# OEmiliatanO/Unpaired-Multimodal-Learning

Measured on AMD Instinct MI355X. Metric: samples/sec (img+text feats) UML head fine-tune, batch 4096, 1/2/4/8 GPU, higher is better.
Workload: dtype bf16; 1 GPU; cfg2 ImageNet-1k CLIP-ViT-B/16 features (d=512) + unpaired CUPL text, linear head C=1000, 4096 img + 4096 txt rows/step/GPU, scale 100, zero-shot init, AdamW lr 1e-3 wd 0.01, warm-up 50 + cosine 12800; n_img_rows=1281167, n_txt_rows=29940, global_batch=8192, parallelism=dp1, dp_stepping=single gpu, precision_mode=bf16, order_rng=device, steps_per_call=25

## Files before the change

### include/umlh.h

```cpp
#ifndef UMLH_H
#define UMLH_H

#include <stdint.h>

#ifdef __cplusplus
extern "C" {
#endif

#define UMLH_OK              0
#define UMLH_E_INVALID      -1
#define UMLH_E_UNBOUND      -2
#define UMLH_E_HIP          -3
#define UMLH_E_NOGPU        -4

#define UMLH_OPT_SGD   0
#define UMLH_OPT_ADAM  1
#define UMLH_OPT_ADAMW 2

#define UMLH_PREC_FP32 0
#define UMLH_PREC_BF16 1

typedef struct umlh_handle_s* umlh_handle_t;

typedef struct {
// ... 186 lines not shown
int  umlh_encoder_stack_backward(const umlh_enc_layer_t* cfg, int32_t n_layers, const float* const* P, const float* h0,
                                 const int64_t* lengths, const float* saved, const float* h, const float* dh_out, float* scratch,
                                 float* const* G, float* dh, float* dh0, void* stream);

typedef struct umlh_enc_plan_s* umlh_enc_plan_t;
uint64_t umlh_encoder_plan_floats(const umlh_enc_layer_t* cfg, int32_t n_layers);
int  umlh_encoder_plan_create(const umlh_enc_layer_t* cfg, int32_t n_layers, const float* const* P, int32_t has_lengths,
                              float* workspace, umlh_enc_plan_t* out);
int  umlh_encoder_plan_offsets(umlh_enc_plan_t plan, uint64_t offsets[6]);
int  umlh_encoder_plan_forward(umlh_enc_plan_t plan, uint64_t seed, void* stream);
int  umlh_encoder_plan_backward(umlh_enc_plan_t plan, void* stream);
void umlh_encoder_plan_destroy(umlh_enc_plan_t plan);

int  umlh_random_permutation(int64_t n, uint64_t seed, int64_t* out, void* stream);

int  umlh_optimizer_step(int32_t optimizer, float* param, const float* grad, float* m, float* v, int64_t n,
                         double lr, int64_t step, double beta1, double beta2, double eps, double momentum,
                         double weight_decay, void* stream);
int  umlh_optimizer_step_multi(int32_t optimizer, int32_t n_tensors, float* const* params, const float* const* grads,
                               float* const* m, float* const* v, const int64_t* n, double lr, int64_t step, double beta1,
                               double beta2, double eps, double momentum, double weight_decay, void* stream);


uint64_t umlh_align_scratch_bytes(int64_t n, int32_t d_a, int32_t d_b, int32_t topk, int32_t splits);
int  umlh_align_knn(const float* x, int64_t n, int32_t d, int32_t ldx, int32_t topk, int32_t splits, int32_t* knn,
                    float* scores, void* scratch, uint64_t scratch_bytes, void* stream);
int  umlh_align_mutual_knn(const int32_t* knn_a, const int32_t* knn_b, int64_t n, int32_t topk, double* out, void* scratch,
                           uint64_t scratch_bytes, void* stream);
int  umlh_align_cka(const float* a, int32_t lda, int32_t d_a, const float* b, int32_t ldb, int32_t d_b, int64_t n,
                    int32_t splits, double* out4, void* scratch, uint64_t scratch_bytes, void* stream);
// ... 138 lines not shown
```

### unpaired-multimodal-learning_amd/csrc/umlh_common.h

```cpp
#pragma once
#include <hip/hip_runtime.h>
#include <stdint.h>
#include "umlh.h"
#include <cstdlib>

typedef float f32x16 __attribute__((ext_vector_type(16)));
typedef float f32x4v __attribute__((ext_vector_type(4)));

constexpr int UMLH_MULTI_OPT_MAX = 48;

constexpr int KT = 16;

static inline int env_int(const char* name, int def) {
    const char* e = getenv(name);
    return e ? atoi(e) : def;
}
#if defined(__HIPCC__)
__device__ __forceinline__ void store_wt_f32(float* p, float v) {
    asm volatile("global_store_dword %0, %1, off sc1" ::"v"(p), "v"(v) : "memory");
}
__device__ __forceinline__ void store_out_f32x4(float* p, f32x4v v, int plain) {
    if (plain) *reinterpret_cast<f32x4v*>(p) = v;
    else asm volatile("global_store_dwordx4 %0, %1, off sc1" ::"v"(p), "v"(v) : "memory");
}
// ... 153 lines not shown
    int   M, N, K, lda, ldo, k_chunk, k_switch, k_valid1, k_valid2, nsplit;
    int   nsplit1;
    const int64_t* a_rows;
    int   bcs;
    void* out16;
    long long slab_stride;
    unsigned long long* stamps;
};

constexpr int UMLH_MULTI_REDUCE_MAX = 16;
struct ReduceDesc { const float* src; float* dst; long long stride; long long n; int ns; int blk0; };
struct MultiReduceArgs {
    ReduceDesc d[UMLH_MULTI_REDUCE_MAX]; int count;
    const float* s_num; const float* s_den; float s_mul;
};

struct OptArgs {
    int   kind;
    float lr, decay;
    float neg_step_size;
    float bc2_sqrt;
    float beta1, one_m_beta1, beta2, one_m_beta2, eps, momentum, wd;
    int   plain;
    int   x3;
};

struct FinalizeArgs {
    const float* partials;
    int   nb0, nb1;
    float inv_rows0, inv_rows1;
// ... 211 lines not shown
```

### unpaired-multimodal-learning_amd/csrc/umlh_kernels_f32.hip

```cpp
#include "umlh_common.h"
#include "umlh_launch.h"
#include <cstdlib>

#ifdef UMLH_ABLATIONS
#define UMLH_ABL(cond) (cond)
#else
#define UMLH_ABL(cond) (false)
#endif

__device__ __forceinline__ f32x4v load4_guard(const float* p, int lim, bool vec_ok) {
    f32x4v v = {0.f, 0.f, 0.f, 0.f};
    if (lim >= 4 && vec_ok) {
        v = *reinterpret_cast<const f32x4v*>(p);
    } else {
        if (lim > 0) v[0] = p[0];
        if (lim > 1) v[1] = p[1];
        if (lim > 2) v[2] = p[2];
        if (lim > 3) v[3] = p[3];
    }
    return v;
}

template <int CTW, int WC, int MODE>
__global__ __launch_bounds__(512) void fwd_ce_f32(FwdArgs a) {
// ... 1395 lines not shown
    for (int j = tid; j < d; j += 256) {
        float mean = count > 0 ? zsum[j] / (float)count : 0.f;
        zsum[j] = mean;
        ss += mean * mean;
    }
    redn[tid] = ss;
    __syncthreads();
    for (int off = 128; off > 0; off >>= 1) {
        if (tid < off) redn[tid] += redn[tid + off];
        __syncthreads();
    }
    float nrm = fmaxf(sqrtf(redn[0]), 1e-12f);
    for (int j = tid; j < d; j += 256) w[(size_t)c * d + j] = zsum[j] / nrm;
}

__device__ __forceinline__ unsigned mix32(unsigned x) {
    x ^= x >> 16; x *= 0x7feb352dU; x ^= x >> 15; x *= 0x846ca68bU; x ^= x >> 16;
    return x;
}

__global__ __launch_bounds__(256) void feistel_perm_kernel(long long n, unsigned long long seed, int half,
                                                           long long* __restrict__ out) {
    long long i = (long long)blockIdx.x * 256 + threadIdx.x;
    if (i >= n) return;
    const unsigned long long mask = (1ULL << half) - 1ULL;
    const unsigned k0 = (unsigned)seed, k1 = (unsigned)(seed >> 32);
    unsigned long long x = (unsigned long long)i;
    do {
        unsigned long long L = x >> half, R = x & mask;
#pragma unroll
        for (int r = 0; r < 4; ++r) {
            unsigned long long F = (unsigned long long)mix32((unsigned)R * 0x9e3779b1U + (r & 1 ? k1 : k0) + 0x85ebca6bU * (unsigned)r +
                                                               (unsigned)(R >> 32)) & mask;
            unsigned long long nl = R;
            R = L ^ F;
            L = nl;
        }
        x = (L << half) | R;
    } while (x >= (unsigned long long)n);
    out[i] = (long long)x;
}

__global__ __launch_bounds__(256) void w_shadow32_kernel(const float* __restrict__ w, float* __restrict__ dst, int C, int K, int cpad) {
    const long long q = (long long)blockIdx.x * 256 + threadIdx.x;
    const int tiles = cpad / 32;
    const long long total = (long long)(K / 16) * tiles * 128;
    if (q >= total) return;
    const int half = (int)(q & 1), lane = (int)((q >> 1) & 63);
    const int tile = (int)((q >> 7) % tiles), c = (int)((q >> 7) / tiles);
    const int cls = tile * 32 + (lane & 31);
    f32x4v v = {0.f, 0.f, 0.f, 0.f};
    if (cls < C) v = *reinterpret_cast<const f32x4v*>(w + (size_t)cls * K + c * 16 + 8 * (lane >> 5) + 4 * half);
    *reinterpret_cast<f32x4v*>(dst + q * 4) = v;
}

// ... 165 lines not shown
    long long n4 = (long long)hf->C * hf->K / 4;
    int blocks = (int)((n4 + 255) / 256) + 1;
    DiagArgs d = *dg;
    if (d.dst && (!d.part || !d.ticket)) return (int)hipErrorInvalidValue;
    if (d.n_slabs_img > hf->n_slabs) d.n_slabs_img = hf->n_slabs;
    OptArgs oc = hf->o;
    oc.plain = umlh_plain_stores();
    oc.x3 = umlh_f32_x3();
    hipLaunchKernelGGL(head_step_kernel, dim3(blocks), dim3(256), 0, stream, hf->slabs, hf->n_slabs, hf->slab_stride, hf->C, hf->K,
                       hf->p, hf->m, hf->v, oc, hf->shadow, hf->cpad, hf->f, hf->grad_out, d, shadow32);
    return (int)hipGetLastError();
}

int umlh_launch_feistel_perm(long long n, unsigned long long seed, long long* out, hipStream_t stream) {
    if (n <= 0) return 0;
    int bits = 1;
    while ((1LL << bits) < n) ++bits;
    int half = (bits + 1) / 2;
    hipLaunchKernelGGL(feistel_perm_kernel, dim3((unsigned)((n + 255) / 256)), dim3(256), 0, stream, n, seed, half, out);
    return (int)hipGetLastError();
}

int umlh_launch_finalize(const FinalizeArgs* f, hipStream_t stream) {
    hipLaunchKernelGGL(finalize_kernel, dim3(1), dim3(256), 0, stream, *f);
    return (int)hipGetLastError();
}

int umlh_launch_zero_shot(const float* feats, const int64_t* labels, long long n, int d, int C, float* w,
                          hipStream_t stream) {
    size_t sm = sizeof(float) * (size_t)(d + 256);
    hipLaunchKernelGGL(zero_shot_kernel, dim3(C), dim3(256), sm, stream, feats, labels, n, d, w);
    return (int)hipGetLastError();
}

// ... 2 lines not shown
```

### unpaired-multimodal-learning_amd/csrc/umlh_launch.h

```cpp
#pragma once
#include <atomic>
#include "umlh_common.h"
#include "umlh_micro.h"

inline long long align_up(long long x) { return (x + 255) / 256 * 256; }
template <class T>
inline T* at(void* scratch, long long off) { return reinterpret_cast<T*>(static_cast<char*>(scratch) + off); }

template <auto Kernel>
__attribute__((visibility("hidden"))) int raise_lds_limit(int bytes) {
    static std::atomic<unsigned long long> done{0};
    int dev = 0;
    hipError_t e = hipGetDevice(&dev);
    if (e != hipSuccess) return (int)e;
    if (!((done.load(std::memory_order_acquire) >> (dev & 63)) & 1ULL)) {
        e = hipFuncSetAttribute(reinterpret_cast<const void*>(Kernel), hipFuncAttributeMaxDynamicSharedMemorySize, bytes);
        if (e != hipSuccess) return (int)e;
        done.fetch_or(1ULL << (dev & 63), std::memory_order_release);
    }
    return 0;
}

extern "C" {
int umlh_launch_w_shadow32(const float* w, float* dst, int C, int K, int cpad, hipStream_t stream);
int umlh_f32_fwd_config(int C, int* ctw, int* wc);
int umlh_f32_launch_fwd(const FwdArgs* a, int ctw, int wc, int grid, hipStream_t stream);
int umlh_f32_launch_gemm(const GemmArgs* g, int ta, int tb, int splits, hipStream_t stream);
int umlh_f32_launch_gemm_enc(const GemmArgs* g, int ta, int tb, int splits, hipStream_t stream);
int umlh_launch_reduce_update(int mode, const float* slabs, int n_slabs, long long slab_stride, long long n, float* grad_out,
                              float* p, float* m, float* v, const OptArgs* o, long long frozen_lo, long long frozen_hi,
                              hipStream_t stream);
int umlh_launch_multi_opt(int n, float* const* p, const float* const* g, float* const* m, float* const* v, const long long* cnt,
                          const OptArgs* o, hipStream_t stream);
int umlh_launch_head_step(const HeadFuse* hf, const DiagArgs* dg, float* shadow32, hipStream_t stream);
int umlh_launch_feistel_perm(long long n, unsigned long long seed, long long* out, hipStream_t stream);
int umlh_launch_finalize(const FinalizeArgs* f, hipStream_t stream);
int umlh_launch_zero_shot(const float* feats, const int64_t* labels, long long n, int d, int C, float* w, hipStream_t stream);
int umlh_launch_to_bf16(const float* src, void* dst, long long n, hipStream_t stream);
int umlh_launch_iota(long long* dst, long long n, hipStream_t stream);
int umlh_launch_w_shadow(const float* w, void* dst, int C, int K, int cpad, hipStream_t stream);
int umlh_bf16_fwd_ts(int wc, int stw);
int umlh_bf16_launch_fwd_q(const FwdArgsB* a, int nq, int tiles, hipStream_t stream);
int umlh_bf16_launch_fwd(const FwdArgsB* a, int ctw, int wc, int stw, int grid, hipStream_t stream);
int umlh_bf16_launch_transpose_shadow(const float* src, int R, int Cc, int ldd, void* dst, int mode, hipStream_t stream);
int umlh_bf16_step_tasks(int nfwd, int M, int N, int splits, long long n_head, int with_head);
int umlh_bf16_launch_step(const FwdArgsB* a, int ctw, int wc, int nfwd, const DwArgsB* g, int splits, unsigned* claim,
                          unsigned long long* done, unsigned* status, unsigned epoch, int ts, int total_cols,
                          const HeadFuse* hf, unsigned long long* timeline, int cus, int lazy, hipStream_t stream);
int umlh_bf16_launch_dw(const DwArgsB* g, int splits, int am, int om, hipStream_t stream);
int umlh_micro_chunking(int d, int* nch, int* cw);
// ... 143 lines not shown
```

### unpaired-multimodal-learning_amd/csrc/umlh_ops.cpp

```cpp
#include <hip/hip_runtime.h>
#include <algorithm>
#include <cmath>
#include <cstring>

#include "umlh_host.h"
#include "umlh_launch.h"

static const int64_t ROWS_END = (int64_t)1 << 31;
static const int64_t ALIGN_MAX_ROWS = (int64_t)1 << 30;
static const int LIST_MAX_K = 24;

static_assert(sizeof(long long) == sizeof(int64_t), "the launchers' long long is the ABI's int64_t");
static inline const long long* ll(const int64_t* p) { return reinterpret_cast<const long long*>(p); }
static inline long long* ll(int64_t* p) { return reinterpret_cast<long long*>(p); }

static const char SCRATCH_OF[] = "%s: scratch of %llu bytes, %llu needed";
static const char SCRATCH_BYTES_EQ[] = "%s: scratch_bytes=%llu, %llu needed";
static int check_scratch(const char* who, const void* scratch, uint64_t scratch_bytes, uint64_t need, unsigned align,
                         const char* size_fmt = SCRATCH_OF) {
    if (scratch_bytes < need) return fail(UMLH_E_INVALID, size_fmt, who, (unsigned long long)scratch_bytes, (unsigned long long)need);
    if (align && (reinterpret_cast<uintptr_t>(scratch) & (align - 1)) != 0)
        return fail(UMLH_E_INVALID, "%s: scratch must be %u-byte aligned", who, align);
    return UMLH_OK;
}
// ... 233 lines not shown
                            int32_t Z, int32_t H, float p, uint64_t seed, float* dqkv, void* stream) {
    if (!qkv || !lse || !dctx || !dqkv || B < 1 || !(p >= 0.f && p < 1.f))
        return fail(UMLH_E_INVALID, "umlh_attention_backward: bad arguments");
    if (T < 1 || T > 128 || H < 1 || Z % H != 0 || Z / H > 64)
        return fail(UMLH_E_INVALID, "umlh_attention_backward: T=%d Z=%d H=%d outside the kernel's envelope", T, Z, H);
    HIPCHK(umlh_enc_launch_attention_bwd(qkv, lengths, lse, dctx, T, B, Z, H, p, seed, nullptr, dqkv, (hipStream_t)stream), "attention_bwd");
    return UMLH_OK;
}

int umlh_random_permutation(int64_t n, uint64_t seed, int64_t* out, void* stream) {
    if (n < 0 || (n > 0 && !out)) return fail(UMLH_E_INVALID, "umlh_random_permutation: bad arguments");
    HIPCHK(umlh_launch_feistel_perm(n, seed, ll(out), (hipStream_t)stream), "feistel perm");
    return UMLH_OK;
}

static OptArgs standalone_opt(int32_t optimizer, double lr, int64_t step, double beta1, double beta2, double eps, double momentum,
                              double weight_decay) {
    umlh_config_t c;
    memset(&c, 0, sizeof(c));
    c.optimizer = optimizer; c.beta1 = beta1; c.beta2 = beta2; c.eps = eps; c.momentum = momentum; c.weight_decay = weight_decay;
    umlh_hyper_t hy;
    memset(&hy, 0, sizeof(hy));
    hy.lr = lr; hy.step = step;
    return make_opt(c, hy);
}

int umlh_optimizer_step(int32_t optimizer, float* param, const float* grad, float* m, float* v, int64_t n, double lr,
                        int64_t step, double beta1, double beta2, double eps, double momentum, double weight_decay,
                        void* stream) {
    if (optimizer < UMLH_OPT_SGD || optimizer > UMLH_OPT_ADAMW)
// ... 630 lines not shown
```

### unpaired-multimodal-learning_amd/engine/datasets/utils.py

```python
from __future__ import annotations

import torch


class TextTensorDataset(torch.utils.data.Dataset):

    def __init__(self, input_tensor, label_tensor, eot_indices, n_shots=None):
        self.input_tensor, self.label_tensor, self.eot_indices = input_tensor, label_tensor, eot_indices
        if isinstance(n_shots, int):
            keep = self._select_n_shots(label_tensor, n_shots)
            if isinstance(input_tensor, list):
                self.input_tensor = [input_tensor[i] for i in keep.tolist()]
            else:
                self.input_tensor = input_tensor[keep]
            self.label_tensor, self.eot_indices = label_tensor[keep], eot_indices[keep]
            print(f"=> Using {n_shots} text shots per class, with total of {len(self)} samples")
        elif isinstance(n_shots, str) and n_shots.lower() == "average":
            self.input_tensor, self.label_tensor, self.eot_indices = self._average_features(
                input_tensor, label_tensor, eot_indices)
            print(f"=> Averaging text features per class, with total of {len(self)} samples")
        elif n_shots is not None:
            raise ValueError("n_shots must be an int, None, or 'average'")

    @staticmethod
# ... 71 lines not shown
        f, y = self.table.features[idx], self.table.labels[idx]
        if self.kind == "image":
            return {"img": f, "label": y, "index": idx}
        eot = self.table.extra[idx] if isinstance(self.table.extra, torch.Tensor) else torch.zeros_like(y)
        return (f, y, eot)

    def __iter__(self):
        for idx in self.iter_index():
            yield self.pack(idx)


class _IndexIter:
    def __init__(self, loader: FeatureLoader):
        self.loader = loader
        torch.empty((), dtype=torch.int64).random_(generator=loader.generator)
        self.order = None
        self.pos = 0

    def __iter__(self):
        return self

    def __next__(self):
        ld = self.loader
        n, bs = len(ld.table), ld.batch_size
        if self.order is None:
            if ld.shuffle:
                seed = int(torch.empty((), dtype=torch.int64).random_(generator=ld.generator).item())
                if ld.order_rng == "device":
                    import umlh
                    self.order = umlh.random_permutation(n, seed, ld.table.device)
                else:
                    g = torch.Generator()
                    g.manual_seed(seed)
                    self.order = torch.randperm(n, generator=g).to(ld.table.device, non_blocking=True)
            else:
                self.order = torch.arange(n, dtype=torch.int64, device=ld.table.device)
        if self.pos >= n or (ld.drop_last and self.pos + bs > n):
            raise StopIteration
        idx = self.order[self.pos:self.pos + bs]
        self.pos += bs
        return idx

    def remaining(self):
        if self.order is None:
            return 0
        ld = self.loader
        n, bs = len(ld.table), ld.batch_size
        left = n - self.pos
        return max(0, left // bs if ld.drop_last else (left + bs - 1) // bs)

    def take_span(self, k):
        ld = self.loader
        n, bs = len(ld.table), ld.batch_size
        end = min(n, self.pos + k * bs)
        idx = self.order[self.pos:end]
        sizes = [bs] * ((end - self.pos) // bs)
        if (end - self.pos) % bs:
            sizes.append((end - self.pos) % bs)
        assert len(sizes) == k
        self.pos = end
        return idx, sizes
```

### unpaired-multimodal-learning_amd/finetune.py

```python
from __future__ import annotations

import os
import sys
import threading
from types import SimpleNamespace
from typing import Optional

import torch

import umlh
from engine.datasets.utils import FeatureLoader, FeatureTable, TextTensorDataset
from engine.models.head import UML, UMLClip
from engine.optimizer.default import HYPER_DICT
from engine.optimizer.optim import build_optimizer
from engine.optimizer.scheduler import build_lr_scheduler
from feature_capture import FeatureCapture
from metrics import AlignmentMetrics, cka, mknn

EVAL_FREQ = 100


def fetch_next(loader, loader_iter):
    try:
        batch = next(loader_iter)
# ... 32 lines not shown

    def __init__(self, loader, device, kind, precision="fp32"):
        self.loader, self.device, self.kind, self.precision = loader, device, kind, precision
        self.indexed = hasattr(loader, "iter_index")
        self._make_iter = loader.iter_index if self.indexed else loader.__iter__
        self.it = self._make_iter()

    @property
    def capacity(self):
        return int(getattr(self.loader, "batch_size", None) or 4096)

    def next_index(self):
        idx, self.it = fetch_next(_Reiter(self._make_iter), self.it)
        return idx

    def remaining(self):
        return self.it.remaining() if self.indexed and hasattr(self.it, "remaining") else 0

    def take_span(self, k):
        return self.it.take_span(k)

    def table(self, precision):
        t = self.loader.table
        return (t.features, t.labels, t.features_bf16()) if precision == "bf16" else (t.features, t.labels)

    def save(self):
        it = self.it
        return it, getattr(it, "order", None), getattr(it, "pos", None)

    def restore(self, st):
        self.it = st[0]
        if st[2] is not None:
            self.it.order, self.it.pos = st[1], st[2]

    def next(self) -> umlh.RowBatch:
        batch, self.it = fetch_next(_Reiter(self._make_iter), self.it)
        if self.indexed:
            t = self.loader.table
            return umlh.RowBatch(t.features, t.labels, batch,
                                 feats_bf16=t.features_bf16() if self.precision == "bf16" else None)
        if self.kind == "image":
            x, y = batch["img"], batch["label"]
        else:
            x, y = batch[0], batch[1]
        return umlh.RowBatch(x.to(self.device, torch.float32).contiguous(), y.to(self.device, torch.int64).contiguous())


class _Reiter:
# ... 34 lines not shown
              "reference does", file=sys.stderr)


def _block_end(i, max_iters, eval_freq):
    return i if i % eval_freq == 0 else min(max_iters - 1, (i // eval_freq + 1) * eval_freq)


def _draw_block(img_src, txt_src, n):
    bi = [] if img_src is not None else None
    bt = [] if txt_src is not None else None
    k = 0
    while k < n:
        span = min([n - k] + [src.remaining() for src in (img_src, txt_src) if src is not None])
        if span == 0:
            if img_src is not None:
                bi.append(img_src.next_index())
            if txt_src is not None:
                bt.append(txt_src.next_index())
            k += 1
        else:
            if img_src is not None:
                bi.append(img_src.take_span(span))
            if txt_src is not None:
                bt.append(txt_src.take_span(span))
            k += span
    return bi, bt


def _rewind_point(img_src, txt_src, optimizer, scheduler):
    gens = []
    for src in (img_src, txt_src):
        g = getattr(src.loader, "generator", None) if src is not None else None
        if src is not None and all(g is not q for q, _ in gens):
# ... 687 lines not shown
```

### unpaired-multimodal-learning_amd/umlh/__init__.py

```python
from ._lib import (UmlhError, build_library, lib_path, load_library, OPT_IDS, PREC_IDS,
                   N_SCALARS, S_LOSS_IMG, S_LOSS_TXT, S_ACC_IMG, S_ACC_TXT, S_GSCALE_IMG, S_GSCALE_TXT,
                   S_CORRECT, S_LOSS_SUM, S_GRAD_DOT, S_GRAD_N2_IMG, S_GRAD_N2_TXT, S_GRAD_AGREE, N_CORE_SCALARS)
from .head_engine import (HeadEngine, RowBatch, column_sums, gather_rows, grad_diagnostics, optimizer_step,
                          optimizer_step_multi,
                          random_permutation, to_bf16, train_steps_grouped)
from .dp import DataParallelStepper
from . import align
from . import probe
from .probe import KNeighborsProbe, LogisticProbe, masked_mean
from . import spectral
from .spectral import effective_rank, effective_rank_seq, principal_subspace, svdvals
from .align import svcca, svcca_terms
from . import capture
from .capture import class_index, class_stats, paired_cosine, seq_compact
from . import stepstats
from .stepstats import seq_step_stats
from . import rollout
from .rollout import rollout_rows, seq_spectrum
from . import report
from .report import class_report, topk_classes


def host_cpu_budget() -> int:
    import os
# ... 29 lines not shown
```

### unpaired-multimodal-learning_amd/umlh/_lib.py

```python
from __future__ import annotations

import ctypes as C
import os
import subprocess
import sys

_HERE = os.path.dirname(os.path.abspath(__file__))
_PKG = os.path.dirname(_HERE)
_ROOT = os.path.dirname(_PKG)
_CSRC = os.path.join(_PKG, "csrc")
_INCLUDE = os.path.join(_ROOT, "include")
_SO = os.path.join(_HERE, "libumlh.so")

OPT_IDS = {"sgd": 0, "adam": 1, "adamw": 2}
PREC_IDS = {"fp32": 0, "bf16": 1}
(S_LOSS_IMG, S_LOSS_TXT, S_ACC_IMG, S_ACC_TXT, S_GSCALE_IMG, S_GSCALE_TXT, S_CORRECT, S_LOSS_SUM,
 S_GRAD_DOT, S_GRAD_N2_IMG, S_GRAD_N2_TXT, S_GRAD_AGREE) = range(12)
N_CORE_SCALARS = 8
N_SCALARS = 12

SOURCES = ["umlh_p2p.hip", "umlh_kernels_f32.hip", "umlh_kernels_bf16.hip", "umlh_kernels_micro.hip", "umlh_kernels_seq.hip", "umlh_kernels_enc.hip", "umlh_kernels_align.hip", "umlh_kernels_align_ext.hip", "umlh_kernels_probe.hip", "umlh_kernels_knn.hip", "umlh_kernels_spectral.hip", "umlh_kernels_capture.hip", "umlh_kernels_stepstats.hip", "umlh_kernels_rollout.hip", "umlh_kernels_classstats.hip", "umlh_kernels_evalreport.hip", "umlh_kernels_outlier.hip", "umlh_api.cpp", "umlh_ops.cpp", "umlh_encoder.cpp"]


class UmlhError(RuntimeError):
# ... 10 lines not shown

class Buffers(C.Structure):
    _fields_ = [(n, C.c_void_p) for n in ("w_head", "m_head", "v_head", "w_proj", "m_proj", "v_proj",
                                          "scales", "m_scales", "v_scales", "workspace")] + \
               [("workspace_bytes", C.c_uint64)]


class Batch(C.Structure):
    _fields_ = [("feats", C.c_void_p), ("labels", C.c_void_p), ("index", C.c_void_p),
                ("rows", C.c_int32), ("global_rows", C.c_int32), ("feats_bf16", C.c_void_p)]


class Stream(C.Structure):
    _fields_ = [("feats", C.c_void_p), ("feats_bf16", C.c_void_p), ("labels", C.c_void_p), ("index", C.c_void_p),
                ("offsets", C.POINTER(C.c_int32))]


ALLREDUCE_FN = C.CFUNCTYPE(C.c_int, C.c_void_p, C.c_void_p, C.c_uint64, C.c_void_p)
COMM_ID_BYTES = 128


class GroupItem(C.Structure):
    _fields_ = [("handle", C.c_void_p), ("img", C.POINTER(Stream)), ("txt", C.POINTER(Stream)),
                ("lr", C.POINTER(C.c_double)), ("first_step", C.c_int64), ("alpha", C.c_float), ("img_alpha", C.c_float),
                ("scalars_out", C.c_void_p)]


class EncLayer(C.Structure):
    _fields_ = [("T", C.c_int32), ("B", C.c_int32), ("Z", C.c_int32), ("H", C.c_int32), ("d_ff", C.c_int32),
                ("p", C.c_float), ("eps", C.c_float), ("seed", C.c_uint64), ("seed_device", C.c_void_p)]
# ... 72 lines not shown
        "umlh_attention_forward": (rc, (vp, vp, i32, i32, i32, i32, f32, u64, vp, vp, vp)),
        "umlh_attention_backward": (rc, (vp, vp, vp, vp, i32, i32, i32, i32, f32, u64, vp, vp)),
        "umlh_encoder_layer_saved_floats": (u64, (enc,)),
        "umlh_encoder_layer_scratch_floats": (u64, (enc,)),
        "umlh_encoder_layer_forward": (rc, (enc, pv, vp, vp, vp, vp, vp, vp)),
        "umlh_encoder_layer_backward": (rc, (enc, pv, vp, vp, vp, vp, vp, pv, vp, vp)),
        "umlh_encoder_stack_forward": (rc, (enc, i32, pv, vp, vp, vp, vp, vp, vp)),
        "umlh_encoder_stack_backward": (rc, (enc, i32, pv, vp, vp, vp, vp, vp, vp, pv, vp, vp, vp)),
        "umlh_encoder_plan_floats": (u64, (enc, i32)),
        "umlh_encoder_plan_create": (rc, (enc, i32, pv, i32, vp, pv)),
        "umlh_encoder_plan_offsets": (rc, (vp, P(u64))),
        "umlh_encoder_plan_forward": (rc, (vp, u64, vp)),
        "umlh_encoder_plan_backward": (rc, (vp, vp)),
        "umlh_encoder_plan_destroy": (None, (vp,)),
        "umlh_random_permutation": (rc, (i64, u64, vp, vp)),
        "umlh_optimizer_step": (rc, (i32, vp, vp, vp, vp, i64, f64, i64, f64, f64, f64, f64, f64, vp)),
        "umlh_optimizer_step_multi": (rc, (i32, i32, pv, pv, pv, pv, P(i64), f64, i64, f64, f64, f64, f64, f64, vp)),
        "umlh_align_scratch_bytes": (u64, (i64, i32, i32, i32, i32)),
        "umlh_align_knn": (rc, (vp, i64, i32, i32, i32, i32, vp, vp, vp, u64, vp)),
        "umlh_align_mutual_knn": (rc, (vp, vp, i64, i32, vp, vp, u64, vp)),
        "umlh_align_cka": (rc, (vp, i32, i32, vp, i32, i32, i64, i32, vp, vp, u64, vp)),
        "umlh_align_ext_scratch_bytes": (u64, (i32, i64, i32, i32, i32, i32)),
        "umlh_align_cka_unbiased": (rc, (vp, i32, i32, vp, i32, i32, i64, i32, vp, vp, u64, vp)),
        "umlh_align_cka_rbf": (rc, (vp, i32, i32, vp, i32, i32, i64, f64, i32, i32, vp, vp, u64, vp)),
        "umlh_align_cknna": (rc, (vp, vp, vp, vp, i64, i32, vp, vp, u64, vp)),
        "umlh_align_list_stats": (rc, (vp, vp, i64, i32, vp, vp, vp, u64, vp)),
        "umlh_masked_mean": (rc, (vp, i32, i32, i32, i64, i64, vp, vp, i32, vp)),
        "umlh_probe_scratch_bytes": (u64, (i64, i32, i32)),
        "umlh_probe_column_stats": (rc, (vp, i64, i32, i32, vp, vp, u64, vp)),
        "umlh_probe_fit": (rc, (vp, i64, i32, i32, vp, vp, i32, f64, i32, f64, vp, vp, vp, vp, u64, vp)),
# ... 84 lines not shown
```

### unpaired-multimodal-learning_amd/umlh/head_engine.py

```python
from __future__ import annotations

import ctypes as C
from dataclasses import dataclass
from typing import Optional

import torch

from . import _lib
from ._glue import ptr, ptr_array, stream
from ._lib import Batch, Buffers, Config, Hyper, OPT_IDS, PREC_IDS, N_SCALARS, Stream, UmlhError, check


ENQUEUE_LOCK = None


@dataclass
class RowBatch:
    feats: torch.Tensor
    labels: torch.Tensor
    index: Optional[torch.Tensor] = None
    rows: Optional[int] = None
    global_rows: Optional[int] = None
    feats_bf16: Optional[torch.Tensor] = None

# ... 205 lines not shown
        parts, sizes = [], []
        for b in batches:
            if isinstance(b, tuple):
                parts.append(b[0])
                sizes.extend(b[1])
            else:
                parts.append(b)
                sizes.append(b.numel())
        if len(sizes) != n:
            raise UmlhError("train_steps: one index vector per step required")
        offs_np = np.zeros(n + 1, dtype=np.int32)
        np.cumsum(np.asarray(sizes, dtype=np.int32), out=offs_np[1:])
        largest = int(np.diff(offs_np).max()) if n else 0
        if largest > cap:
            raise UmlhError(f"train_steps: batch of {largest} rows exceeds capacity {cap}")
        idx = torch.cat(parts) if len(parts) > 1 else parts[0].contiguous()
        if idx.numel() != int(offs_np[n]):
            raise UmlhError("train_steps: index slices do not match their batch sizes")
        offs = offs_np.ctypes.data_as(C.POINTER(C.c_int32))
        keep = (f, y, f16, idx, offs_np)
        return Stream(ptr(f), ptr(f16), ptr(y), ptr(idx), offs), keep

    def train_steps(self, img_table, img_index_batches, txt_table, txt_index_batches, lrs, first_step: int,
                    alpha: float = 1.0, img_alpha: float = 1.0, scalars_out: Optional[torch.Tensor] = None) -> None:
        self.train_steps_prepared(self.prepare_steps(img_table, img_index_batches, txt_table, txt_index_batches, lrs),
                                  first_step, alpha=alpha, img_alpha=img_alpha, scalars_out=scalars_out)

    def prepare_steps(self, img_table, img_index_batches, txt_table, txt_index_batches, lrs):
        n = len(lrs)
        si, keep_i = self._make_stream(img_table, img_index_batches, self.d_img, self.cfg.max_rows_img, n)
        st, keep_t = self._make_stream(txt_table, txt_index_batches, self.d_shared, self.cfg.max_rows_txt, n)
        lr_arr = (C.c_double * n)(*[float(x) for x in lrs])
        return (n, si, st, lr_arr, keep_i, keep_t)

    def train_steps_prepared(self, prep, first_step: int, alpha: float = 1.0, img_alpha: float = 1.0,
                             scalars_out: Optional[torch.Tensor] = None) -> None:
        n, si, st, lr_arr, keep_i, keep_t = prep
        lock = ENQUEUE_LOCK
        if lock is not None:
            lock.acquire()
        try:
            rc = self.lib.umlh_train_steps(self.handle, self._ref(si), self._ref(st), n, lr_arr, int(first_step),
                                           float(alpha), float(img_alpha), ptr(scalars_out), stream(self.device))
        finally:
            if lock is not None:
                lock.release()
        check(rc, "umlh_train_steps")
        self._keepalive = (keep_i, keep_t)
# ... 172 lines not shown


def train_steps_grouped(jobs, n_steps: int) -> None:
    if not jobs:
        return
    from ._lib import GroupItem
    items = (GroupItem * len(jobs))()
    keep = []
    for j, job in enumerate(jobs):
        e = job["engine"]
        lrs = job["lrs"]
        if len(lrs) != n_steps:
            raise UmlhError("train_steps_grouped: every head needs n_steps learning rates")
        si, ki = e._make_stream(job.get("img_table"), job.get("img_index_batches"), e.d_img, e.cfg.max_rows_img, n_steps)
        st, kt = e._make_stream(job.get("txt_table"), job.get("txt_index_batches"), e.d_shared, e.cfg.max_rows_txt, n_steps)
        lr_arr = (C.c_double * n_steps)(*[float(x) for x in lrs])
        so = job.get("scalars_out")
        items[j] = GroupItem(e.handle, C.pointer(si) if si is not None else None, C.pointer(st) if st is not None else None,
                             lr_arr, int(job["first_step"]), float(job.get("alpha", 1.0)), float(job.get("img_alpha", 1.0)),
                             ptr(so))
        keep.append((si, st, ki, kt, lr_arr, so))
        e._keepalive = (ki, kt)
    e0 = jobs[0]["engine"]
    check(e0.lib.umlh_train_steps_grouped(items, len(jobs), int(n_steps), stream(e0.device)), "umlh_train_steps_grouped")


def grad_diagnostics(scalars, n_elements: int, rows_img: int = 1, rows_txt: int = 1) -> dict:
    import math
    row = [float(x) for x in scalars[:_lib.N_SCALARS].tolist()]
    n2i, n2t = row[_lib.S_GRAD_N2_IMG], row[_lib.S_GRAD_N2_TXT]
# ... 64 lines not shown
    lib = _lib.load_library()
    if t.dtype != torch.float32 or not t.is_contiguous() or t.device.type != "cuda":
        raise UmlhError("to_bf16: contiguous fp32 GPU tensor required")
    out = torch.empty(t.shape, dtype=torch.bfloat16, device=t.device)
    st = stream(t.device)
    check(lib.umlh_to_bf16(ptr(t), ptr(out), t.numel(), st), "umlh_to_bf16")
    return out


def random_permutation(n: int, seed: int, device) -> torch.Tensor:
    lib = _lib.load_library()
    out = torch.empty(n, dtype=torch.int64, device=device)
    st = stream(out.device)
    check(lib.umlh_random_permutation(int(n), int(seed) & 0xFFFFFFFFFFFFFFFF, ptr(out), st), "umlh_random_permutation")
    return out
```

Baseline: 192.0 million samples/s.

## Generate per-block batch indices on device from lazy epoch-order spans

Replaces materialised epoch permutations and host-side slicing and torch.cat of index tensors with lazy IndexSpan descriptors. A single index_block kernel evaluates the Feistel permutation, table lookup or iota for every span directly into the stream's index buffer. This is meant to remove the separate full-epoch permutation kernel, the slice and concatenate ops and several small launches per call. In exchange it recomputes the Feistel mapping per block and allocates a fresh index tensor on every prepare.

```diff
diff --git a/include/umlh.h b/include/umlh.h
--- a/include/umlh.h
+++ b/include/umlh.h
@@ -224,6 +224,20 @@
 
 int  umlh_random_permutation(int64_t n, uint64_t seed, int64_t* out, void* stream);
 
+#define UMLH_SPAN_FEISTEL 0
+#define UMLH_SPAN_TABLE   1
+#define UMLH_SPAN_IOTA    2
+typedef struct {
+    int32_t kind;
+    int32_t reserved;
+    int64_t n;
+    uint64_t seed;
+    const int64_t* order;
+    int64_t start, count;
+} umlh_index_span_t;
+int  umlh_index_block(const umlh_index_span_t* img_spans, int32_t n_img_spans, int64_t* img_out,
+                      const umlh_index_span_t* txt_spans, int32_t n_txt_spans, int64_t* txt_out, void* stream);
+
 int  umlh_optimizer_step(int32_t optimizer, float* param, const float* grad, float* m, float* v, int64_t n,
                          double lr, int64_t step, double beta1, double beta2, double eps, double momentum,
                          double weight_decay, void* stream);
diff --git a/unpaired-multimodal-learning_amd/csrc/umlh_common.h b/unpaired-multimodal-learning_amd/csrc/umlh_common.h
--- a/unpaired-multimodal-learning_amd/csrc/umlh_common.h
+++ b/unpaired-multimodal-learning_amd/csrc/umlh_common.h
@@ -191,6 +191,11 @@
     ReduceDesc d[UMLH_MULTI_REDUCE_MAX]; int count;
     const float* s_num; const float* s_den; float s_mul;
 };
+
+constexpr int UMLH_INDEX_SPANS_MAX = 32;
+struct IndexSpanDesc { const long long* order; long long* dst; long long n; unsigned long long seed; long long start; long long count;
+                       int kind; int half; int blk0; int pad; };
+struct IndexBlockArgs { IndexSpanDesc s[UMLH_INDEX_SPANS_MAX]; int count; };
 
 struct OptArgs {
     int   kind;
diff --git a/unpaired-multimodal-learning_amd/csrc/umlh_feistel.h b/unpaired-multimodal-learning_amd/csrc/umlh_feistel.h
--- /dev/null
+++ b/unpaired-multimodal-learning_amd/csrc/umlh_feistel.h
@@ -0,0 +1,32 @@
+#pragma once
+#include <hip/hip_runtime.h>
+
+inline int feistel_half(long long n) {
+    int bits = 1;
+    while ((1LL << bits) < n) ++bits;
+    return (bits + 1) / 2;
+}
+
+__device__ __forceinline__ unsigned mix32(unsigned x) {
+    x ^= x >> 16; x *= 0x7feb352dU; x ^= x >> 15; x *= 0x846ca68bU; x ^= x >> 16;
+    return x;
+}
+
+__device__ __forceinline__ long long feistel_index(long long i, long long n, unsigned long long seed, int half) {
+    const unsigned long long mask = (1ULL << half) - 1ULL;
+    const unsigned k0 = (unsigned)seed, k1 = (unsigned)(seed >> 32);
+    unsigned long long x = (unsigned long long)i;
+    do {
+        unsigned long long L = x >> half, R = x & mask;
+#pragma unroll
+        for (int r = 0; r < 4; ++r) {
+            unsigned long long F = (unsigned long long)mix32((unsigned)R * 0x9e3779b1U + (r & 1 ? k1 : k0) + 0x85ebca6bU * (unsigned)r +
+                                                               (unsigned)(R >> 32)) & mask;
+            unsigned long long nl = R;
+            R = L ^ F;
+            L = nl;
+        }
+        x = (L << half) | R;
+    } while (x >= (unsigned long long)n);
+    return (long long)x;
+}
diff --git a/unpaired-multimodal-learning_amd/csrc/umlh_kernels_f32.hip b/unpaired-multimodal-learning_amd/csrc/umlh_kernels_f32.hip
--- a/unpaired-multimodal-learning_amd/csrc/umlh_kernels_f32.hip
+++ b/unpaired-multimodal-learning_amd/csrc/umlh_kernels_f32.hip
@@ -1,5 +1,6 @@
 #include "umlh_common.h"
 #include "umlh_launch.h"
+#include "umlh_feistel.h"
 #include <cstdlib>
 
 #ifdef UMLH_ABLATIONS
@@ -1433,31 +1434,24 @@
     for (int j = tid; j < d; j += 256) w[(size_t)c * d + j] = zsum[j] / nrm;
 }
 
-__device__ __forceinline__ unsigned mix32(unsigned x) {
-    x ^= x >> 16; x *= 0x7feb352dU; x ^= x >> 15; x *= 0x846ca68bU; x ^= x >> 16;
-    return x;
-}
-
 __global__ __launch_bounds__(256) void feistel_perm_kernel(long long n, unsigned long long seed, int half,
                                                            long long* __restrict__ out) {
     long long i = (long long)blockIdx.x * 256 + threadIdx.x;
     if (i >= n) return;
-    const unsigned long long mask = (1ULL << half) - 1ULL;
-    const unsigned k0 = (unsigned)seed, k1 = (unsigned)(seed >> 32);
-    unsigned long long x = (unsigned long long)i;
-    do {
-        unsigned long long L = x >> half, R = x & mask;
-#pragma unroll
-        for (int r = 0; r < 4; ++r) {
-            unsigned long long F = (unsigned long long)mix32((unsigned)R * 0x9e3779b1U + (r & 1 ? k1 : k0) + 0x85ebca6bU * (unsigned)r +
-                                                               (unsigned)(R >> 32)) & mask;
-            unsigned long long nl = R;
-            R = L ^ F;
-            L = nl;
-        }
-        x = (L << half) | R;
-    } while (x >= (unsigned long long)n);
-    out[i] = (long long)x;
+    out[i] = feistel_index(i, n, seed, half);
+}
+
+__global__ __launch_bounds__(256) void index_block_kernel(IndexBlockArgs a) {
+    int s = 0;
+    while (s + 1 < a.count && (int)blockIdx.x >= a.s[s + 1].blk0) ++s;
+    const IndexSpanDesc& d = a.s[s];
+    const long long j = (long long)((int)blockIdx.x - d.blk0) * 256 + threadIdx.x;
+    if (j >= d.count) return;
+    const long long i = d.start + j;
+    long long id = i;
+    if (d.kind == UMLH_SPAN_FEISTEL) id = feistel_index(i, d.n, d.seed, d.half);
+    else if (d.kind == UMLH_SPAN_TABLE) id = d.order[i];
+    d.dst[j] = id;
 }
 
 __global__ __launch_bounds__(256) void w_shadow32_kernel(const float* __restrict__ w, float* __restrict__ dst, int C, int K, int cpad) {
@@ -1653,10 +1647,21 @@
 
 int umlh_launch_feistel_perm(long long n, unsigned long long seed, long long* out, hipStream_t stream) {
     if (n <= 0) return 0;
-    int bits = 1;
-    while ((1LL << bits) < n) ++bits;
-    int half = (bits + 1) / 2;
-    hipLaunchKernelGGL(feistel_perm_kernel, dim3((unsigned)((n + 255) / 256)), dim3(256), 0, stream, n, seed, half, out);
+    hipLaunchKernelGGL(feistel_perm_kernel, dim3((unsigned)((n + 255) / 256)), dim3(256), 0, stream, n, seed, feistel_half(n), out);
+    return (int)hipGetLastError();
+}
+
+int umlh_launch_index_block(IndexBlockArgs* a, hipStream_t stream) {
+    long long blocks = 0;
+    for (int i = 0; i < a->count; ++i) {
+        IndexSpanDesc& d = a->s[i];
+        d.half = d.kind == UMLH_SPAN_FEISTEL ? feistel_half(d.n) : 0;
+        d.blk0 = (int)blocks;
+        blocks += (d.count + 255) / 256;
+        if (blocks > 0x7fffffffLL) return (int)hipErrorInvalidValue;
+    }
+    if (blocks == 0) return 0;
+    hipLaunchKernelGGL(index_block_kernel, dim3((unsigned)blocks), dim3(256), 0, stream, *a);
     return (int)hipGetLastError();
 }
 
diff --git a/unpaired-multimodal-learning_amd/csrc/umlh_launch.h b/unpaired-multimodal-learning_amd/csrc/umlh_launch.h
--- a/unpaired-multimodal-learning_amd/csrc/umlh_launch.h
+++ b/unpaired-multimodal-learning_amd/csrc/umlh_launch.h
@@ -34,6 +34,7 @@
                           const OptArgs* o, hipStream_t stream);
 int umlh_launch_head_step(const HeadFuse* hf, const DiagArgs* dg, float* shadow32, hipStream_t stream);
 int umlh_launch_feistel_perm(long long n, unsigned long long seed, long long* out, hipStream_t stream);
+int umlh_launch_index_block(IndexBlockArgs* a, hipStream_t stream);
 int umlh_launch_finalize(const FinalizeArgs* f, hipStream_t stream);
 int umlh_launch_zero_shot(const float* feats, const int64_t* labels, long long n, int d, int C, float* w, hipStream_t stream);
 int umlh_launch_to_bf16(const float* src, void* dst, long long n, hipStream_t stream);
diff --git a/unpaired-multimodal-learning_amd/csrc/umlh_ops.cpp b/unpaired-multimodal-learning_amd/csrc/umlh_ops.cpp
--- a/unpaired-multimodal-learning_amd/csrc/umlh_ops.cpp
+++ b/unpaired-multimodal-learning_amd/csrc/umlh_ops.cpp
@@ -271,6 +271,54 @@
     return UMLH_OK;
 }
 
+static int check_index_spans(const char* who, const char* side, const umlh_index_span_t* spans, int32_t n_spans, const int64_t* out,
+                             int64_t* total) {
+    *total = 0;
+    if (n_spans < 0 || (n_spans > 0 && !spans)) return fail(UMLH_E_INVALID, "%s: %s: %d spans without a span array", who, side, n_spans);
+    for (int i = 0; i < n_spans; ++i) {
+        const umlh_index_span_t& s = spans[i];
+        if (s.kind < UMLH_SPAN_FEISTEL || s.kind > UMLH_SPAN_IOTA) return fail(UMLH_E_INVALID, "%s: %s span %d: unknown kind %d", who, side, i, s.kind);
+        if (s.n < 0 || s.start < 0 || s.count < 0 || s.start > s.n || s.count > s.n - s.start)
+            return fail(UMLH_E_INVALID, "%s: %s span %d: start=%lld count=%lld outside an order of n=%lld rows", who, side, i,
+                        (long long)s.start, (long long)s.count, (long long)s.n);
+        if (s.kind == UMLH_SPAN_FEISTEL && s.n > ((int64_t)1 << 62))
+            return fail(UMLH_E_INVALID, "%s: %s span %d: n=%lld rows (a Feistel order holds at most 2^62)", who, side, i, (long long)s.n);
+        if (s.kind == UMLH_SPAN_TABLE && s.count > 0 && !s.order) return fail(UMLH_E_INVALID, "%s: %s span %d: a TABLE span needs its order", who, side, i);
+        *total += s.count;
+        if (*total >= ROWS_END) return fail(UMLH_E_INVALID, "%s: %s: more than 2^31 - 1 ids in one block", who, side);
+    }
+    if (*total > 0 && !out) return fail(UMLH_E_INVALID, "%s: %s: %lld ids and no destination", who, side, (long long)*total);
+    return UMLH_OK;
+}
+
+int umlh_index_block(const umlh_index_span_t* img_spans, int32_t n_img_spans, int64_t* img_out, const umlh_index_span_t* txt_spans,
+                     int32_t n_txt_spans, int64_t* txt_out, void* stream) {
+    const char* who = "umlh_index_block";
+    int64_t total_img = 0, total_txt = 0;
+    RC(check_index_spans(who, "image", img_spans, n_img_spans, img_out, &total_img));
+    RC(check_index_spans(who, "text", txt_spans, n_txt_spans, txt_out, &total_txt));
+    IndexBlockArgs a;
+    memset(&a, 0, sizeof(a));
+    const umlh_index_span_t* side[2] = {img_spans, txt_spans};
+    const int32_t n_side[2] = {n_img_spans, n_txt_spans};
+    int64_t* dst_side[2] = {img_out, txt_out};
+    for (int m = 0; m < 2; ++m) {
+        long long* dst = ll(dst_side[m]);
+        for (int i = 0; i < n_side[m]; ++i) {
+            const umlh_index_span_t& s = side[m][i];
+            if (s.count == 0) continue;
+            a.s[a.count++] = IndexSpanDesc{ll(s.order), dst, s.n, s.seed, s.start, s.count, s.kind, 0, 0, 0};
+            dst += s.count;
+            if (a.count == UMLH_INDEX_SPANS_MAX) {
+                HIPCHK(umlh_launch_index_block(&a, (hipStream_t)stream), who);
+                a.count = 0;
+            }
+        }
+    }
+    if (a.count > 0) HIPCHK(umlh_launch_index_block(&a, (hipStream_t)stream), who);
+    return UMLH_OK;
+}
+
 static OptArgs standalone_opt(int32_t optimizer, double lr, int64_t step, double beta1, double beta2, double eps, double momentum,
                               double weight_decay) {
     umlh_config_t c;
diff --git a/unpaired-multimodal-learning_amd/engine/datasets/utils.py b/unpaired-multimodal-learning_amd/engine/datasets/utils.py
--- a/unpaired-multimodal-learning_amd/engine/datasets/utils.py
+++ b/unpaired-multimodal-learning_amd/engine/datasets/utils.py
@@ -109,35 +109,56 @@
     def __init__(self, loader: FeatureLoader):
         self.loader = loader
         torch.empty((), dtype=torch.int64).random_(generator=loader.generator)
-        self.order = None
+        self.epoch = None
         self.pos = 0
 
     def __iter__(self):
         return self
 
-    def __next__(self):
+    @property
+    def order(self):
+        return None if self.epoch is None else self.epoch.tensor()
+
+    @order.setter
+    def order(self, value):
+        if value is None:
+            self.epoch = None
+        elif self.epoch is None or self.epoch._order is not value:
+            import umlh
+            self.epoch = umlh.EpochOrder.table(value)
+
+    def _begin_epoch(self):
+        import umlh
+        ld = self.loader
+        n, dev = len(ld.table), ld.table.device
+        if ld.shuffle:
+            seed = int(torch.empty((), dtype=torch.int64).random_(generator=ld.generator).item())
+            if ld.order_rng == "device":
+                self.epoch = umlh.EpochOrder.permutation(n, seed, dev)
+            else:
+                g = torch.Generator()
+                g.manual_seed(seed)
+                self.epoch = umlh.EpochOrder.table(torch.randperm(n, generator=g).to(dev, non_blocking=True))
+        else:
+            self.epoch = umlh.EpochOrder.identity(n, dev)
+
+    def next_span(self):
+        import umlh
         ld = self.loader
         n, bs = len(ld.table), ld.batch_size
-        if self.order is None:
-            if ld.shuffle:
-                seed = int(torch.empty((), dtype=torch.int64).random_(generator=ld.generator).item())
-                if ld.order_rng == "device":
-                    import umlh
-                    self.order = umlh.random_permutation(n, seed, ld.table.device)
-                else:
-                    g = torch.Generator()
-                    g.manual_seed(seed)
-                    self.order = torch.randperm(n, generator=g).to(ld.table.device, non_blocking=True)
-            else:
-                self.order = torch.arange(n, dtype=torch.int64, device=ld.table.device)
+        if self.epoch is None:
+            self._begin_epoch()
         if self.pos >= n or (ld.drop_last and self.pos + bs > n):
             raise StopIteration
-        idx = self.order[self.pos:self.pos + bs]
+        span = umlh.IndexSpan(self.epoch, self.pos, min(bs, n - self.pos))
         self.pos += bs
-        return idx
+        return span
+
+    def __next__(self):
+        return self.next_span().tensor()
 
     def remaining(self):
-        if self.order is None:
+        if self.epoch is None:
             return 0
         ld = self.loader
         n, bs = len(ld.table), ld.batch_size
@@ -145,13 +166,14 @@
         return max(0, left // bs if ld.drop_last else (left + bs - 1) // bs)
 
     def take_span(self, k):
+        import umlh
         ld = self.loader
         n, bs = len(ld.table), ld.batch_size
         end = min(n, self.pos + k * bs)
-        idx = self.order[self.pos:end]
+        span = umlh.IndexSpan(self.epoch, self.pos, end - self.pos)
         sizes = [bs] * ((end - self.pos) // bs)
         if (end - self.pos) % bs:
             sizes.append((end - self.pos) % bs)
         assert len(sizes) == k
         self.pos = end
-        return idx, sizes
+        return span, sizes
diff --git a/unpaired-multimodal-learning_amd/finetune.py b/unpaired-multimodal-learning_amd/finetune.py
--- a/unpaired-multimodal-learning_amd/finetune.py
+++ b/unpaired-multimodal-learning_amd/finetune.py
@@ -70,6 +70,15 @@
         idx, self.it = fetch_next(_Reiter(self._make_iter), self.it)
         return idx
 
+    def next_span(self):
+        if not hasattr(self.it, "next_span"):
+            return self.next_index()
+        try:
+            return self.it.next_span()
+        except StopIteration:
+            self.it = self._make_iter()
+            return self.it.next_span()
+
     def remaining(self):
         return self.it.remaining() if self.indexed and hasattr(self.it, "remaining") else 0
 
@@ -82,12 +91,12 @@
 
     def save(self):
         it = self.it
-        return it, getattr(it, "order", None), getattr(it, "pos", None)
+        return it, getattr(it, "epoch", None), getattr(it, "pos", None)
 
     def restore(self, st):
         self.it = st[0]
         if st[2] is not None:
-            self.it.order, self.it.pos = st[1], st[2]
+            self.it.epoch, self.it.pos = st[1], st[2]
 
     def next(self) -> umlh.RowBatch:
         batch, self.it = fetch_next(_Reiter(self._make_iter), self.it)
@@ -152,9 +161,9 @@
         span = min([n - k] + [src.remaining() for src in (img_src, txt_src) if src is not None])
         if span == 0:
             if img_src is not None:
-                bi.append(img_src.next_index())
+                bi.append(img_src.next_span())
             if txt_src is not None:
-                bt.append(txt_src.next_index())
+                bt.append(txt_src.next_span())
             k += 1
         else:
             if img_src is not None:
diff --git a/unpaired-multimodal-learning_amd/umlh/__init__.py b/unpaired-multimodal-learning_amd/umlh/__init__.py
--- a/unpaired-multimodal-learning_amd/umlh/__init__.py
+++ b/unpaired-multimodal-learning_amd/umlh/__init__.py
@@ -1,8 +1,8 @@
 from ._lib import (UmlhError, build_library, lib_path, load_library, OPT_IDS, PREC_IDS,
                    N_SCALARS, S_LOSS_IMG, S_LOSS_TXT, S_ACC_IMG, S_ACC_TXT, S_GSCALE_IMG, S_GSCALE_TXT,
                    S_CORRECT, S_LOSS_SUM, S_GRAD_DOT, S_GRAD_N2_IMG, S_GRAD_N2_TXT, S_GRAD_AGREE, N_CORE_SCALARS)
-from .head_engine import (HeadEngine, RowBatch, column_sums, gather_rows, grad_diagnostics, optimizer_step,
-                          optimizer_step_multi,
+from .head_engine import (EpochOrder, HeadEngine, IndexSpan, RowBatch, column_sums, gather_rows, grad_diagnostics,
+                          index_block, optimizer_step, optimizer_step_multi,
                           random_permutation, to_bf16, train_steps_grouped)
 from .dp import DataParallelStepper
 from . import align
diff --git a/unpaired-multimodal-learning_amd/umlh/_lib.py b/unpaired-multimodal-learning_amd/umlh/_lib.py
--- a/unpaired-multimodal-learning_amd/umlh/_lib.py
+++ b/unpaired-multimodal-learning_amd/umlh/_lib.py
@@ -48,6 +48,14 @@
 class Stream(C.Structure):
     _fields_ = [("feats", C.c_void_p), ("feats_bf16", C.c_void_p), ("labels", C.c_void_p), ("index", C.c_void_p),
                 ("offsets", C.POINTER(C.c_int32))]
+
+
+SPAN_FEISTEL, SPAN_TABLE, SPAN_IOTA = range(3)
+
+
+class IndexSpanDesc(C.Structure):
+    _fields_ = [("kind", C.c_int32), ("reserved", C.c_int32), ("n", C.c_int64), ("seed", C.c_uint64), ("order", C.c_void_p),
+                ("start", C.c_int64), ("count", C.c_int64)]
 
 
 ALLREDUCE_FN = C.CFUNCTYPE(C.c_int, C.c_void_p, C.c_void_p, C.c_uint64, C.c_void_p)
@@ -150,6 +158,7 @@
         "umlh_encoder_plan_backward": (rc, (vp, vp)),
         "umlh_encoder_plan_destroy": (None, (vp,)),
         "umlh_random_permutation": (rc, (i64, u64, vp, vp)),
+        "umlh_index_block": (rc, (P(IndexSpanDesc), i32, vp, P(IndexSpanDesc), i32, vp, vp)),
         "umlh_optimizer_step": (rc, (i32, vp, vp, vp, vp, i64, f64, i64, f64, f64, f64, f64, f64, vp)),
         "umlh_optimizer_step_multi": (rc, (i32, i32, pv, pv, pv, pv, P(i64), f64, i64, f64, f64, f64, f64, f64, vp)),
         "umlh_align_scratch_bytes": (u64, (i64, i32, i32, i32, i32)),
diff --git a/unpaired-multimodal-learning_amd/umlh/head_engine.py b/unpaired-multimodal-learning_amd/umlh/head_engine.py
--- a/unpaired-multimodal-learning_amd/umlh/head_engine.py
+++ b/unpaired-multimodal-learning_amd/umlh/head_engine.py
@@ -243,12 +243,28 @@
         largest = int(np.diff(offs_np).max()) if n else 0
         if largest > cap:
             raise UmlhError(f"train_steps: batch of {largest} rows exceeds capacity {cap}")
-        idx = torch.cat(parts) if len(parts) > 1 else parts[0].contiguous()
-        if idx.numel() != int(offs_np[n]):
+        if sum(int(p.numel()) for p in parts) != int(offs_np[n]):
             raise UmlhError("train_steps: index slices do not match their batch sizes")
+        idx = fill = None
+        if len(parts) == 1 and isinstance(parts[0], torch.Tensor):
+            idx = parts[0].contiguous()
+        else:
+            fill = (_span_descs(parts, self.device), int(offs_np[n]))
         offs = offs_np.ctypes.data_as(C.POINTER(C.c_int32))
-        keep = (f, y, f16, idx, offs_np)
+        keep = [f, y, f16, idx, offs_np, fill]
         return Stream(ptr(f), ptr(f16), ptr(y), ptr(idx), offs), keep
+
+    def _fill_index(self, si, keep_i, st, keep_t) -> None:
+        fills = []
+        for s, k in ((si, keep_i), (st, keep_t)):
+            if k is None or k[5] is None:
+                fills.append(None)
+                continue
+            k[3] = torch.empty(k[5][1], dtype=torch.int64, device=self.device)
+            s.index = k[3].data_ptr()
+            fills.append((k[5][0], k[3]))
+        if fills[0] is not None or fills[1] is not None:
+            _index_block_launch(self.lib, fills[0], fills[1], self.device)
 
     def train_steps(self, img_table, img_index_batches, txt_table, txt_index_batches, lrs, first_step: int,
                     alpha: float = 1.0, img_alpha: float = 1.0, scalars_out: Optional[torch.Tensor] = None) -> None:
@@ -259,8 +275,13 @@
         n = len(lrs)
         si, keep_i = self._make_stream(img_table, img_index_batches, self.d_img, self.cfg.max_rows_img, n)
         st, keep_t = self._make_stream(txt_table, txt_index_batches, self.d_shared, self.cfg.max_rows_txt, n)
+        self._fill_index(si, keep_i, st, keep_t)
         lr_arr = (C.c_double * n)(*[float(x) for x in lrs])
         return (n, si, st, lr_arr, keep_i, keep_t)
+
+    @staticmethod
+    def prepared_index(prep):
+        return tuple(None if k is None else (k[3], k[4]) for k in (prep[4], prep[5]))
 
     def train_steps_prepared(self, prep, first_step: int, alpha: float = 1.0, img_alpha: float = 1.0,
                              scalars_out: Optional[torch.Tensor] = None) -> None:
@@ -463,6 +484,7 @@
             raise UmlhError("train_steps_grouped: every head needs n_steps learning rates")
         si, ki = e._make_stream(job.get("img_table"), job.get("img_index_batches"), e.d_img, e.cfg.max_rows_img, n_steps)
         st, kt = e._make_stream(job.get("txt_table"), job.get("txt_index_batches"), e.d_shared, e.cfg.max_rows_txt, n_steps)
+        e._fill_index(si, ki, st, kt)
         lr_arr = (C.c_double * n_steps)(*[float(x) for x in lrs])
         so = job.get("scalars_out")
         items[j] = GroupItem(e.handle, C.pointer(si) if si is not None else None, C.pointer(st) if st is not None else None,
@@ -557,3 +579,92 @@
     st = stream(out.device)
     check(lib.umlh_random_permutation(int(n), int(seed) & 0xFFFFFFFFFFFFFFFF, ptr(out), st), "umlh_random_permutation")
     return out
+
+
+class EpochOrder:
+    __slots__ = ("kind", "n", "seed", "device", "_order")
+
+    def __init__(self, kind: int, n: int, device, seed: int = 0, order: Optional[torch.Tensor] = None):
+        if kind == _lib.SPAN_TABLE and order is None:
+            raise UmlhError("EpochOrder: a TABLE order needs its tensor")
+        self.kind, self.n, self.seed, self.device, self._order = kind, int(n), int(seed) & 0xFFFFFFFFFFFFFFFF, device, order
+
+    @classmethod
+    def permutation(cls, n, seed, device):
+        return cls(_lib.SPAN_FEISTEL, n, device, seed=seed)
+
+    @classmethod
+    def table(cls, order: torch.Tensor):
+        return cls(_lib.SPAN_TABLE, order.numel(), order.device, order=order)
+
+    @classmethod
+    def identity(cls, n, device):
+        return cls(_lib.SPAN_IOTA, n, device)
+
+    def tensor(self) -> torch.Tensor:
+        if self._order is None:
+            self._order = (random_permutation(self.n, self.seed, self.device) if self.kind == _lib.SPAN_FEISTEL
+                           else torch.arange(self.n, dtype=torch.int64, device=self.device))
+        return self._order
+
+
+class IndexSpan:
+    __slots__ = ("epoch", "start", "count")
+
+    def __init__(self, epoch: EpochOrder, start: int, count: int):
+        if start < 0 or count < 0 or start + count > epoch.n:
+            raise UmlhError(f"IndexSpan: start={start} count={count} outside an order of {epoch.n} rows")
+        self.epoch, self.start, self.count = epoch, int(start), int(count)
+
+    def numel(self) -> int:
+        return self.count
+
+    def tensor(self) -> torch.Tensor:
+        return self.epoch.tensor()[self.start:self.start + self.count]
+
+
+def _span_descs(parts, device):
+    arr = (_lib.IndexSpanDesc * len(parts))()
+    keep = []
+    for k, p in enumerate(parts):
+        if isinstance(p, IndexSpan):
+            e = p.epoch
+            order = e.tensor() if e.kind == _lib.SPAN_TABLE else None
+            arr[k] = _lib.IndexSpanDesc(e.kind, 0, e.n, e.seed, order.data_ptr() if order is not None else None, p.start, p.count)
+        else:
+            order = p if p.is_contiguous() else p.contiguous()
+            arr[k] = _lib.IndexSpanDesc(_lib.SPAN_TABLE, 0, order.numel(), 0, order.data_ptr(), 0, order.numel())
+        if order is not None:
+            if order.dtype != torch.int64 or order.device.type != torch.device(device).type or not order.is_contiguous():
+                raise UmlhError("index vectors must be contiguous int64 tensors on the engine's device")
+            keep.append(order)
+    return arr, keep
+
+
+def _index_block_launch(lib, fill_img, fill_txt, device) -> None:
+    def side(fill):
+        if fill is None:
+            return None, 0, None
+        (arr, _), out = fill
+        return arr, len(arr), ptr(out)
+    ai, ni, oi = side(fill_img)
+    at, nt, ot = side(fill_txt)
+    check(lib.umlh_index_block(ai, ni, oi, at, nt, ot, stream(device)), "umlh_index_block")
+
+
+def index_block(img_parts, txt_parts, device, out=(None, None)):
+    lib = _lib.load_library()
+    device = torch.device(device)
+    fills = []
+    for parts, dst in zip((img_parts, txt_parts), out):
+        if parts is None:
+            fills.append(None)
+            continue
+        total = sum(int(p.numel()) for p in parts)
+        if dst is None:
+            dst = torch.empty(total, dtype=torch.int64, device=device)
+        elif dst.dtype != torch.int64 or not dst.is_contiguous() or dst.numel() != total or dst.device.type != device.type:
+            raise UmlhError(f"index_block: out must be a contiguous int64 device tensor of {total} ids")
+        fills.append((_span_descs(parts, device), dst))
+    _index_block_launch(lib, fills[0], fills[1], device)
+    return tuple(None if f is None else f[1] for f in fills)
```

New measurement: 195.1 million samples/s, median of 6. 1.6% higher.
